# Wuziyi616/multi_part_assembly

Measured on AMD Instinct MI355X. Metric: train-step parts/sec (BxP) at N=1000 pts, higher is better.
Workload: dtype f32

## Files before the change

### multi_part_assembly_amd/csrc/gate_nn.hip

```cpp
#include "assembly_internal.h"
#include "common.h"
#include "gate_common.h"

namespace mpa {
namespace {

using gate::f32x16;
typedef unsigned long long u64;

constexpr int kGW = 4;
constexpr int kGQ = 64 * kGW;
constexpr int kGT = 1024;
constexpr int kGTiles = kGT / 32;
constexpr float kGKappa = 6.0e-5f;
constexpr float kGMaxNorm = 1e30f;

__device__ __forceinline__ float g_dist3(float dx, float dy, float dz) { return (dx * dx + dy * dy) + dz * dz; }
__device__ __forceinline__ u64 g_key(float d, unsigned idx) { return ((u64)__float_as_uint(d) << 32) | idx; }

struct GateArgs {
  const float* a;
  const float* b;
  const float* valids;
  int na, nb, tiles;
  int* idx32[2];
  float* tile_sums;
  float* dist[2];
  long long* idx64[2];
  int M;
};

template <bool LOSS>
__global__ __launch_bounds__(kGQ, 3) void gate_nn_kernel(const GateArgs g) {
  __shared__ uint4 panel[2][kGT];
  __shared__ float4 raw[kGT + kGT / 32];
  __shared__ float red[kGW], redm[kGW];
  const int m = blockIdx.x / g.tiles, tile = blockIdx.x % g.tiles, dir = blockIdx.y;
  if (g.valids != nullptr && g.valids[m] == 0.0f) return;
  const int nq = dir == 0 ? g.na : g.nb, nt = dir == 0 ? g.nb : g.na;
  const int qbase = tile * kGQ;
  if (qbase >= nq) return;
  const float* qa = (dir == 0 ? g.a : g.b) + 3LL * m * nq;
  const float* tb = (dir == 0 ? g.b : g.a) + 3LL * m * nt;
  const int wave = __builtin_amdgcn_readfirstlane((int)(threadIdx.x >> 6)), lane = threadIdx.x & 63;
  const int j = lane & 31, h = lane >> 5;
  const int qi = qbase + (int)threadIdx.x;
  const bool has = qi < nq;
  const int qc = has ? qi : nq - 1;
  const float X = qa[3LL * qc], Y = qa[3LL * qc + 1], Z = qa[3LL * qc + 2];
  float bd = 1e32f;
  int bi = -1;

  auto store = [&]() {
    if (LOSS) {
      if (has) g.idx32[dir][(long long)m * nq + qi] = bi;
      float s = has ? bd : 0.0f;
#pragma unroll
      for (int off = 32; off > 0; off >>= 1) s += __shfl_xor(s, off, 64);
      if (lane == 0) red[wave] = s;
      __syncthreads();
      if (threadIdx.x == 0) {
        float t = 0.0f;
#pragma unroll
        for (int w = 0; w < kGW; ++w) t += red[w];
        g.tile_sums[((long long)dir * g.M + m) * g.tiles + tile] = t;
      }
    } else if (has) {
      g.dist[dir][(long long)m * nq + qi] = bd;
      g.idx64[dir][(long long)m * nq + qi] = (long long)bi;
    }
  };
  if (nt == 0) {
    store();
    return;
  }

  float cx = 0.0f, cy = 0.0f, cz = 0.0f;
  {
    const int nc = nt < 16 ? nt : 16;
    for (int t = 0; t < nc; ++t) {
      cx += tb[3 * t];
      cy += tb[3 * t + 1];
      cz += tb[3 * t + 2];
    }
    const float inv = 1.0f / (float)nc;
    cx *= inv, cy *= inv, cz *= inv;
  }

  uint4 bq[2];
  float OX, OY, OZ;
  float mq;
  {
    const float yx = X - cx, yy = Y - cy, yz = Z - cz;
    mq = g_dist3(yx, yy, yz);
    uint4 k0, k1;
    gate::query_column(yx, yy, yz, k0, k1);
    gate::wave_columns(k0, k1, j, h, bq);
    OX = __shfl(X, 32 * (1 - h) + j, 64), OY = __shfl(Y, 32 * (1 - h) + j, 64), OZ = __shfl(Z, 32 * (1 - h) + j, 64);
  }

  const float t0x = tb[0], t0y = tb[1], t0z = tb[2];
  bool same = true;
  float mmax = 0.0f;
  const float nanf_ = __builtin_nanf("");
  auto stage = [&](int chunk) {
    for (int r = threadIdx.x; r < kGT; r += kGQ) {
      const int t = chunk * kGT + r;
      float yx = 0.0f, yy = 0.0f, yz = 0.0f, n = 3.0e38f;
      float4 rw = {nanf_, nanf_, nanf_, 0.0f};
      if (t < nt) {
        const float x = tb[3LL * t], y = tb[3LL * t + 1], z = tb[3LL * t + 2];
        rw = float4{x, y, z, 0.0f};
        same = same && x == t0x && y == t0y && z == t0z;
        yx = x - cx, yy = y - cy, yz = z - cz;
        n = g_dist3(yx, yy, yz);
        mmax = n > mmax || n != n ? n : mmax;
      }
      uint4 p0, p1;
      gate::target_row(yx, yy, yz, n, p0, p1);
      panel[0][r] = p0;
      panel[1][r] = p1;
      raw[r + (r >> 5)] = rw;
    }
  };
  float tm0[kGTiles], tm1[kGTiles];
  float run0 = __builtin_inff(), run1 = __builtin_inff();
  auto bound = [&](int c) {
    const int rows = nt - c * kGT < kGT ? nt - c * kGT : kGT;
    const int nti = (rows + 31) / 32;
    const uint4* pl = &panel[h][j];
#pragma unroll
    for (int t8 = 0; t8 < kGTiles; t8 += 8) {
      if (t8 < nti) {
        uint4 nx = pl[32 * t8];
#pragma unroll
        for (int t = t8; t < t8 + 8; ++t) {
          const gate::bf16x8 a = gate::as_bf16x8(nx);
          if (t + 1 < t8 + 8) nx = pl[32 * (t + 1)];
          const f32x16 z = {0};
          const f32x16 acc0 = __builtin_amdgcn_mfma_f32_32x32x16_bf16(a, gate::as_bf16x8(bq[0]), z, 0, 0, 0);
          const f32x16 acc1 = __builtin_amdgcn_mfma_f32_32x32x16_bf16(a, gate::as_bf16x8(bq[1]), z, 0, 0, 0);
          float x, y;
          gate::min16(acc0, x, y);
          tm0[t] = gate::min3(x, y, __builtin_inff());
          run0 = gate::min3(run0, x, y);
          gate::min16(acc1, x, y);
          tm1[t] = gate::min3(x, y, __builtin_inff());
          run1 = gate::min3(run1, x, y);
          __builtin_amdgcn_sched_barrier(0);
        }
      } else {
#pragma unroll
        for (int t = t8; t < t8 + 8; ++t) tm0[t] = tm1[t] = __builtin_inff();
      }
    }
  };
  const int chunks = (nt + kGT - 1) / kGT;
  stage(0);
  const bool all_same = __syncthreads_and(same ? 1 : 0) != 0;
  if (chunks == 1 && all_same) {
    const float d = g_dist3(X - t0x, Y - t0y, Z - t0z);
    if (d < 1e32f) {
      bd = d;
      bi = 0;
    }
    store();
    return;
  }
  const u64 none = g_key(1e32f, 0xffffffffu);
  u64 best0 = none, best1 = none;
  float thr0 = 0.0f, thr1 = 0.0f;
  bool wave_exact = false;
  const int sweeps = chunks == 1 ? 1 : 2;
  for (int sw = 0; sw < sweeps; ++sw) {
    const bool last = sw == sweeps - 1;
    for (int c = 0; c < chunks; ++c) {
      if (sw > 0 || c > 0) {
        __syncthreads();
        stage(c);
        __syncthreads();
      }
      bound(c);
      if (!last) continue;
      if (c == 0) {
        float v = mmax;
#pragma unroll
        for (int off = 32; off > 0; off >>= 1) {
          const float o = __shfl_xor(v, off, 64);
          v = o > v || o != o ? o : v;
        }
        if (lane == 0) redm[wave] = v;
        __syncthreads();
        mmax = redm[0];
#pragma unroll
        for (int w = 1; w < kGW; ++w) mmax = redm[w] > mmax || redm[w] != redm[w] ? redm[w] : mmax;
        const float tau0 = gate::min3(run0, __shfl_xor(run0, 32, 64), __builtin_inff());
        const float tau1 = gate::min3(run1, __shfl_xor(run1, 32, 64), __builtin_inff());
        float sl = gate::next_up(gate::next_up(mq + mmax) * (2.0f * kGKappa));
        sl = gate::next_up(sl + 1e-30f);
        const float thr_own = gate::next_up((h ? tau1 : tau0) + sl);
        thr0 = __shfl(thr_own, j, 64), thr1 = __shfl(thr_own, 32 + j, 64);
        const bool risky = has && !(mq <= kGMaxNorm && mmax <= kGMaxNorm);
        wave_exact = __ballot(risky) != 0;
      }
      if (wave_exact) continue;
      unsigned k0 = 0u, k1 = 0u;
#pragma unroll
      for (int t = kGTiles - 1; t >= 0; --t) {
        k0 = (k0 << 1) | (tm0[t] <= thr0 ? 1u : 0u);
        k1 = (k1 << 1) | (tm1[t] <= thr1 ? 1u : 0u);
      }
      while (__ballot((k0 | k1) != 0u)) {
        const bool act = (k0 | k1) != 0u, from1 = k0 == 0u;
        const unsigned mm = from1 ? k1 : k0;
        const int t = act ? __builtin_ctz(mm) : 0;
        k0 = from1 ? k0 : k0 & (k0 - 1u);
        k1 = from1 && act ? k1 & (k1 - 1u) : k1;
        const bool own = from1 == (h == 1);
        const float qx = act ? (own ? X : OX) : nanf_, qy = own ? Y : OY, qz = own ? Z : OZ;
        u64 cur = from1 ? best1 : best0;
        const int row0 = 32 * t + 4 * h;
        const unsigned gidx = (unsigned)(c * kGT + row0);
#pragma unroll
        for (int g2 = 0; g2 < 8; ++g2) {
          const int ro = 8 * (g2 >> 1) + 2 * (g2 & 1);
          const float4 pa = raw[row0 + t + ro], pb = raw[row0 + t + ro + 1];
          const u64 ka = g_key(g_dist3(qx - pa.x, qy - pa.y, qz - pa.z), gidx + ro);
          const u64 kb = g_key(g_dist3(qx - pb.x, qy - pb.y, qz - pb.z), gidx + ro + 1);
          cur = ka < cur ? ka : cur;
          cur = kb < cur ? kb : cur;
        }
        best0 = from1 ? best0 : cur;
        best1 = from1 ? cur : best1;
      }
    }
  }
  if (wave_exact) {
    for (int t = 0; t < nt; ++t) {
      const float d = g_dist3(X - tb[3LL * t], Y - tb[3LL * t + 1], Z - tb[3LL * t + 2]);
      if (d < bd) {
        bd = d;
        bi = t;
      }
    }
  } else {
    const u64 o0 = __shfl_xor(best0, 32, 64), o1 = __shfl_xor(best1, 32, 64);
    const u64 m0 = o0 < best0 ? o0 : best0, m1 = o1 < best1 ? o1 : best1;
    const u64 mine = h ? m1 : m0;
    const unsigned db = (unsigned)(mine >> 32);
    if (db != __float_as_uint(1e32f)) {
      bd = __uint_as_float(db);
      bi = (int)(unsigned)mine;
    }
  }
  store();
}

}

int gate_tiles(int64_t na, int64_t nb) { return (int)(((na > nb ? na : nb) + kGQ - 1) / kGQ); }
bool gate_supported(int64_t na, int64_t nb) { return na >= 1 && nb >= 1 && na <= 32768 && nb <= 32768; }

void launch_gate_part_search(const float* valids, const float* C1, const float* C2, int64_t B, int64_t P, int64_t N,
                             int32_t* idx1, int32_t* idx2, float* tile_sums, hipStream_t s) {
  GateArgs g = {};
  g.a = C1, g.b = C2, g.valids = valids;
  g.na = g.nb = (int)N;
  g.tiles = gate_tiles(N, N);
  g.idx32[0] = idx1, g.idx32[1] = idx2;
  g.tile_sums = tile_sums;
  g.M = (int)(B * P);
  hipLaunchKernelGGL((gate_nn_kernel<true>), dim3((unsigned)(B * P * g.tiles), 2), dim3(kGQ), 0, s, g);
}

void launch_gate_cloud_search(const float* xyz1, const float* xyz2, int64_t batch, int64_t n1, int64_t n2, float* dist1,
                              int64_t* idx1, float* dist2, int64_t* idx2, hipStream_t s) {
  GateArgs g = {};
  g.a = xyz1, g.b = xyz2, g.valids = nullptr;
  g.na = (int)n1, g.nb = (int)n2;
  g.tiles = gate_tiles(n1, n2);
  g.dist[0] = dist1, g.dist[1] = dist2;
  g.idx64[0] = reinterpret_cast<long long*>(idx1), g.idx64[1] = reinterpret_cast<long long*>(idx2);
  g.M = (int)batch;
  hipLaunchKernelGGL((gate_nn_kernel<false>), dim3((unsigned)(batch * g.tiles), 2), dim3(kGQ), 0, s, g);
}

}
```

Baseline: 379,400.

## Compact candidate tile refinements into a block-wide work list for balanced rescoring

Before, each lane walked its own flagged candidate tiles inside a ballot loop, so a wave stayed busy until its slowest lane finished. Now each wave compacts its (query slot, tile, half) candidates into a shared-memory list that reuses the panel buffer. All threads in the block then split that list evenly, and each computes exact distances and merges its result into per-query shared bests with 64-bit atomicMin. If any wave's list would overflow its region, the old per-lane loop runs instead. The cost is extra __syncthreads, shared-memory atomics and bookkeeping in exchange for better load balance across lanes and waves.

```diff
diff --git a/multi_part_assembly_amd/csrc/gate_nn.hip b/multi_part_assembly_amd/csrc/gate_nn.hip
--- a/multi_part_assembly_amd/csrc/gate_nn.hip
+++ b/multi_part_assembly_amd/csrc/gate_nn.hip
@@ -14,6 +14,9 @@
 constexpr int kGTiles = kGT / 32;
 constexpr float kGKappa = 6.0e-5f;
 constexpr float kGMaxNorm = 1e30f;
+constexpr int kGCap = (2 * kGT * 16 - kGQ * 16) / 2;
+constexpr int kGRegion = kGCap / kGW;
+static_assert(kGCap % (8 * kGW) == 0 && kGCap * 2 + kGQ * 16 == 2 * kGT * 16, "list + queries fill the panel exactly");
 
 __device__ __forceinline__ float g_dist3(float dx, float dy, float dz) { return (dx * dx + dy * dy) + dz * dz; }
 __device__ __forceinline__ u64 g_key(float d, unsigned idx) { return ((u64)__float_as_uint(d) << 32) | idx; }
@@ -35,6 +38,10 @@
   __shared__ uint4 panel[2][kGT];
   __shared__ float4 raw[kGT + kGT / 32];
   __shared__ float red[kGW], redm[kGW];
+  __shared__ u64 bestq[kGQ];
+  __shared__ int wcnt[kGW];
+  unsigned short* const list = reinterpret_cast<unsigned short*>(&panel[0][0]);
+  float4* const qs = reinterpret_cast<float4*>(&panel[0][0]) + kGCap * sizeof(unsigned short) / sizeof(float4);
   const int m = blockIdx.x / g.tiles, tile = blockIdx.x % g.tiles, dir = blockIdx.y;
   if (g.valids != nullptr && g.valids[m] == 0.0f) return;
   const int nq = dir == 0 ? g.na : g.nb, nt = dir == 0 ? g.nb : g.na;
@@ -88,7 +95,6 @@
   }
 
   uint4 bq[2];
-  float OX, OY, OZ;
   float mq;
   {
     const float yx = X - cx, yy = Y - cy, yz = Z - cz;
@@ -96,7 +102,6 @@
     uint4 k0, k1;
     gate::query_column(yx, yy, yz, k0, k1);
     gate::wave_columns(k0, k1, j, h, bq);
-    OX = __shfl(X, 32 * (1 - h) + j, 64), OY = __shfl(Y, 32 * (1 - h) + j, 64), OZ = __shfl(Z, 32 * (1 - h) + j, 64);
   }
 
   const float t0x = tb[0], t0y = tb[1], t0z = tb[2];
@@ -156,6 +161,8 @@
     }
   };
   const int chunks = (nt + kGT - 1) / kGT;
+  const u64 none = g_key(1e32f, 0xffffffffu);
+  bestq[threadIdx.x] = none;
   stage(0);
   const bool all_same = __syncthreads_and(same ? 1 : 0) != 0;
   if (chunks == 1 && all_same) {
@@ -167,8 +174,6 @@
     store();
     return;
   }
-  const u64 none = g_key(1e32f, 0xffffffffu);
-  u64 best0 = none, best1 = none;
   float thr0 = 0.0f, thr1 = 0.0f;
   bool wave_exact = false;
   const int sweeps = chunks == 1 ? 1 : 2;
@@ -203,38 +208,96 @@
         const bool risky = has && !(mq <= kGMaxNorm && mmax <= kGMaxNorm);
         wave_exact = __ballot(risky) != 0;
       }
-      if (wave_exact) continue;
+      if (c > 0) __syncthreads();
       unsigned k0 = 0u, k1 = 0u;
 #pragma unroll
       for (int t = kGTiles - 1; t >= 0; --t) {
         k0 = (k0 << 1) | (tm0[t] <= thr0 ? 1u : 0u);
         k1 = (k1 << 1) | (tm1[t] <= thr1 ? 1u : 0u);
       }
-      while (__ballot((k0 | k1) != 0u)) {
-        const bool act = (k0 | k1) != 0u, from1 = k0 == 0u;
-        const unsigned mm = from1 ? k1 : k0;
-        const int t = act ? __builtin_ctz(mm) : 0;
-        k0 = from1 ? k0 : k0 & (k0 - 1u);
-        k1 = from1 && act ? k1 & (k1 - 1u) : k1;
-        const bool own = from1 == (h == 1);
-        const float qx = act ? (own ? X : OX) : nanf_, qy = own ? Y : OY, qz = own ? Z : OZ;
-        u64 cur = from1 ? best1 : best0;
-        const int row0 = 32 * t + 4 * h;
-        const unsigned gidx = (unsigned)(c * kGT + row0);
-#pragma unroll
-        for (int g2 = 0; g2 < 8; ++g2) {
-          const int ro = 8 * (g2 >> 1) + 2 * (g2 & 1);
-          const float4 pa = raw[row0 + t + ro], pb = raw[row0 + t + ro + 1];
-          const u64 ka = g_key(g_dist3(qx - pa.x, qy - pa.y, qz - pa.z), gidx + ro);
-          const u64 kb = g_key(g_dist3(qx - pb.x, qy - pb.y, qz - pb.z), gidx + ro + 1);
-          cur = ka < cur ? ka : cur;
-          cur = kb < cur ? kb : cur;
-        }
-        best0 = from1 ? best0 : cur;
-        best1 = from1 ? cur : best1;
-      }
-    }
-  }
+      const unsigned slot0 = 64u * (unsigned)wave + (unsigned)j, slot1 = slot0 + 32u;
+      k0 = !wave_exact && qbase + (int)slot0 < nq ? k0 : 0u;
+      k1 = !wave_exact && qbase + (int)slot1 < nq ? k1 : 0u;
+      qs[threadIdx.x] = float4{X, Y, Z, 0.0f};
+      {
+        unsigned a0 = k0, a1 = k1;
+        int pos = 0;
+        for (;;) {
+          const bool act = (a0 | a1) != 0u;
+          const u64 bal = __ballot(act);
+          if (bal == 0ull) break;
+          const bool from1 = a0 == 0u;
+          const unsigned mm = from1 ? a1 : a0;
+          const int p = pos + (int)__builtin_amdgcn_mbcnt_hi((unsigned)(bal >> 32), __builtin_amdgcn_mbcnt_lo((unsigned)bal, 0u));
+          if (act && p < kGRegion)
+            list[wave * kGRegion + p] =
+                (unsigned short)((from1 ? slot1 : slot0) | ((unsigned)__builtin_ctz(mm) << 8) | ((unsigned)h << 13));
+          a0 = from1 ? a0 : a0 & (a0 - 1u);
+          a1 = from1 && act ? a1 & (a1 - 1u) : a1;
+          pos += __popcll(bal);
+        }
+        if (lane == 0) wcnt[wave] = pos;
+      }
+      __syncthreads();
+      const int c0 = __builtin_amdgcn_readfirstlane(wcnt[0]), c1 = __builtin_amdgcn_readfirstlane(wcnt[1]);
+      const int c2 = __builtin_amdgcn_readfirstlane(wcnt[2]), c3 = __builtin_amdgcn_readfirstlane(wcnt[3]);
+      static_assert(kGW == 4, "the regions' counts are read one by one");
+      const int total = c0 + c1 + c2 + c3;
+      if (c0 <= kGRegion && c1 <= kGRegion && c2 <= kGRegion && c3 <= kGRegion) {
+        for (int e = threadIdx.x; e < total; e += kGQ) {
+          int r = e, w = 0;
+          if (r >= c0) r -= c0, w = 1;
+          if (w == 1 && r >= c1) r -= c1, w = 2;
+          if (w == 2 && r >= c2) r -= c2, w = 3;
+          const unsigned ent = list[w * kGRegion + r];
+          const unsigned slot = ent & 255u;
+          const int t = (int)((ent >> 8) & 31u), hh = (int)(ent >> 13);
+          const float4 q = qs[slot];
+          const int row0 = 32 * t + 4 * hh;
+          const unsigned gidx = (unsigned)(c * kGT + row0);
+          u64 cur = none;
+#pragma unroll
+          for (int g2 = 0; g2 < 8; ++g2) {
+            const int ro = 8 * (g2 >> 1) + 2 * (g2 & 1);
+            const float4 pa = raw[row0 + t + ro], pb = raw[row0 + t + ro + 1];
+            const u64 ka = g_key(g_dist3(q.x - pa.x, q.y - pa.y, q.z - pa.z), gidx + ro);
+            const u64 kb = g_key(g_dist3(q.x - pb.x, q.y - pb.y, q.z - pb.z), gidx + ro + 1);
+            cur = ka < cur ? ka : cur;
+            cur = kb < cur ? kb : cur;
+          }
+          atomicMin(&bestq[slot], cur);
+        }
+      } else {
+        u64 best0 = none, best1 = none;
+        while (__ballot((k0 | k1) != 0u)) {
+          const bool act = (k0 | k1) != 0u, from1 = k0 == 0u;
+          const unsigned mm = from1 ? k1 : k0;
+          const int t = act ? __builtin_ctz(mm) : 0;
+          k0 = from1 ? k0 : k0 & (k0 - 1u);
+          k1 = from1 && act ? k1 & (k1 - 1u) : k1;
+          const float4 q = qs[from1 ? slot1 : slot0];
+          const float qx = act ? q.x : nanf_;
+          u64 cur = from1 ? best1 : best0;
+          const int row0 = 32 * t + 4 * h;
+          const unsigned gidx = (unsigned)(c * kGT + row0);
+#pragma unroll
+          for (int g2 = 0; g2 < 8; ++g2) {
+            const int ro = 8 * (g2 >> 1) + 2 * (g2 & 1);
+            const float4 pa = raw[row0 + t + ro], pb = raw[row0 + t + ro + 1];
+            const u64 ka = g_key(g_dist3(qx - pa.x, q.y - pa.y, q.z - pa.z), gidx + ro);
+            const u64 kb = g_key(g_dist3(qx - pb.x, q.y - pb.y, q.z - pb.z), gidx + ro + 1);
+            cur = ka < cur ? ka : cur;
+            cur = kb < cur ? kb : cur;
+          }
+          best0 = from1 ? best0 : cur;
+          best1 = from1 ? cur : best1;
+        }
+        atomicMin(&bestq[slot0], best0);
+        atomicMin(&bestq[slot1], best1);
+      }
+    }
+  }
+  __syncthreads();
   if (wave_exact) {
     for (int t = 0; t < nt; ++t) {
       const float d = g_dist3(X - tb[3LL * t], Y - tb[3LL * t + 1], Z - tb[3LL * t + 2]);
@@ -244,9 +307,9 @@
       }
     }
   } else {
-    const u64 o0 = __shfl_xor(best0, 32, 64), o1 = __shfl_xor(best1, 32, 64);
-    const u64 m0 = o0 < best0 ? o0 : best0, m1 = o1 < best1 ? o1 : best1;
-    const u64 mine = h ? m1 : m0;
+    int slot = (int)threadIdx.x;
+    asm volatile("" : "+v"(slot));
+    const u64 mine = bestq[slot];
     const unsigned db = (unsigned)(mine >> 32);
     if (db != __float_as_uint(1e32f)) {
       bd = __uint_as_float(db);
```

Result: no change. 376,200 (-0.9%).
